# y-scope/pinot

Hardware: AMD Instinct MI355X
Metric: scanned rows/sec + achieved HBM GB/s, filtered SUM on 1B-row segment (higher is better)
Workload: dtype int64

## Files before the change

### pinot_amd/csrc/pg_engine.hip

```cpp
#include <hip/hip_runtime.h>

#include <algorithm>
#include <chrono>
#include <array>
#include <atomic>
#include <condition_variable>
#include <functional>
#include <memory>
#include <cmath>
#include <cstdarg>
#include <cstdio>
#include <cstdlib>
#include <cstring>
#include <limits>
#include <mutex>
#include <string>
#include <thread>
#include <vector>

#include "../../include/pinot_gpu.h"
#include "pg_device.h"
#include "pg_filter_stats.h"
#include "pg_filter_fsm.h"
#include "pg_fsm_kernels.h"
#include "pg_kernels.h"
#include "pg_launch.h"
#include "pg_rank_image.h"
#include "pg_raw_set_table.h"
#include "pg_hll.h"
#include "pg_set_pass_layout.h"
#include "pg_group_plan.h"
#include "pg_chunk_decode.h"

namespace {

using namespace pg;

thread_local std::string g_error;

pg_status fail(pg_status st, const char* fmt, ...) {
  char buf[1024];
  va_list ap;
  va_start(ap, fmt);
  vsnprintf(buf, sizeof(buf), fmt, ap);
  va_end(ap);
  g_error = buf;
  return st;
}

#define HIP_TRY(expr)                                                                                  \
  do {                                                                                                 \
    hipError_t _e = (expr);                                                                            \
    if (_e != hipSuccess)                                                                              \
      return fail(_e == hipErrorOutOfMemory ? PG_ERR_OUT_OF_MEMORY : PG_ERR_DEVICE, "%s failed: %s (%s:%d)", #expr, \
                  hipGetErrorString(_e), __FILE__, __LINE__);                                          \
  } while (0)

struct Engine {
  bool initialized = false;
  std::atomic<uint64_t> epoch{0};
  int device = 0;
  int blocks_per_cu = 0;
  bool raw64_coalesced = true;
  int wide_plane = -1;
  bool partition_stats_cache = true;
  bool partition_packed = true;
  bool plane_async = true;
  bool staged_h2d = true;
  long long exact_stats_docs = 64ll << 20;
  int flags = 0;
  bool use_dma = true;
  int value_plane = -1;
  int tile_steps = 0;
  bool double_buffer = false;
  bool direct_result = true;
  int fold_finalize = -1;
  int fold_one_counter = 1;
  bool poll_result = true;
  bool distinct_lds = true;
  bool collect = false;
  bool chunk_decode_host = false;
  bool percentile_lds = true;
  bool set_lds = true;
  bool lane_skip = true;
  bool batch_blocks_per_cu_forced = false;
  int batch_blocks_per_cu = 4;
  bool scan_raw = true;
  bool scan_raw_set = true;
  int scan_simple_valid = 1;
  int scan_simple_pipe = 1;
  int scan_simple_dma = 1;
  int dma_nt = -1;
  int dma_blocks_per_cu = 0;
  bool scan_simple = true;
  bool scan_sparse = true;
  bool lean_batch = true;
  bool partition_two_level = true;
  bool fsm_perm = true;
  int index_and_waves = 0;
  bool batch_index = true;
  bool index_gather = true;
  bool fsm_fused = true;
  bool fsm_stats = true;
  bool fsm_episodes = true;
  bool plan_cache = true;
  bool group_publish = true;
  bool batch_more = true;
  bool group_one_launch = true;
  bool batch_group = true;
  bool batch_hist = true;
  bool batch_launch = true;
  bool leap2 = true;
  int sparse_lanes = 32;
  bool plane_gcd = true;
  bool scan_private = true;
  bool group_private = true;
  int group_log_replicas = 3;
  bool group_pack = true;
  bool scan_typed_private = true;
  bool scan_narrow_single = true;
  bool scan_narrow = true;
  bool group_partition = true;
  long long partition_min_docs = 1ll << 22;
  unsigned long long group_table_bytes = 64ull << 30;
// ... 1648 lines not shown
  if (dev < 0 || dev >= g_engine.logical_devices) return fail(PG_ERR_INVALID_ARGUMENT, "device %d out of range (have %d)", dev, g_engine.logical_devices);
  g_engine.device = dev;
  g_engine.blocks_per_cu = config ? config->blocks_per_cu : 0;
  g_engine.flags = config ? config->flags : 0;
  const char* nodma = getenv("PINOT_GPU_NO_DMA");
  g_engine.use_dma = !(nodma && nodma[0] == '1');
  const char* vp = getenv("PINOT_GPU_VALUE_PLANE");
  g_engine.value_plane = vp ? atoi(vp) : -1;
  const char* db = getenv("PINOT_GPU_DOUBLE_BUFFER");
  g_engine.double_buffer = db && db[0] == '1';
  const char* drv = getenv("PINOT_GPU_DIRECT_RESULT");
  g_engine.direct_result = !(drv && drv[0] == '0');
  const char* ffz = getenv("PINOT_GPU_FOLD_FINALIZE");
  g_engine.fold_finalize = ffz ? (ffz[0] == '0' ? 0 : 1) : -1;
  const char* foc = getenv("PINOT_GPU_FOLD_ONE_COUNTER");
  g_engine.fold_one_counter = foc ? (foc[0] == '0' ? 0 : 1) : 1;
  const char* prs = getenv("PINOT_GPU_POLL_RESULT");
  g_engine.poll_result = !(prs && prs[0] == '0');
  const char* lsk = getenv("PINOT_GPU_LANE_SKIP");
  g_engine.lane_skip = !(lsk && lsk[0] == '0');
  const char* bbc = getenv("PINOT_GPU_BATCH_BLOCKS_PER_CU");
  g_engine.batch_blocks_per_cu_forced = bbc != nullptr;
  g_engine.batch_blocks_per_cu = (bbc && atoi(bbc) > 0) ? atoi(bbc) : 4;
  const char* ssp = getenv("PINOT_GPU_SCAN_SPARSE");
  g_engine.scan_sparse = !(ssp && ssp[0] == '0');
  const char* ssm = getenv("PINOT_GPU_SCAN_SIMPLE");
  g_engine.scan_simple = !(ssm && ssm[0] == '0');
  const char* ssv = getenv("PINOT_GPU_SCAN_SIMPLE_VALID");
  g_engine.scan_simple_valid = ssv ? (ssv[0] == '0' ? 0 : (ssv[0] == '2' ? 2 : 1)) : 1;
  const char* spp = getenv("PINOT_GPU_SCAN_SIMPLE_PIPE");
  g_engine.scan_simple_pipe = spp ? (spp[0] == '0' ? 0 : (spp[0] == '2' ? 2 : 1)) : 1;
  const char* sdm = getenv("PINOT_GPU_SCAN_SIMPLE_DMA");
  g_engine.scan_simple_dma = sdm ? (sdm[0] == '0' ? 0 : (sdm[0] == '2' ? 2 : 1)) : 1;
  const char* sdn = getenv("PINOT_GPU_SCAN_SIMPLE_DMA_NT");
  g_engine.dma_nt = sdn ? (sdn[0] == '0' ? 0 : 1) : -1;
  const char* sdb = getenv("PINOT_GPU_SCAN_SIMPLE_DMA_BLOCKS_PER_CU");
  g_engine.dma_blocks_per_cu = sdb && atoi(sdb) > 0 ? atoi(sdb) : 0;
  const char* srw = getenv("PINOT_GPU_SCAN_RAW");
  g_engine.scan_raw = !(srw && srw[0] == '0');
  const char* srs = getenv("PINOT_GPU_SCAN_RAW_SET");
  g_engine.scan_raw_set = !(srs && srs[0] == '0');
  const char* bla = getenv("PINOT_GPU_BATCH_LAUNCH");
  g_engine.batch_launch = !(bla && bla[0] == '0');
  auto env_on = [](const char* name) { const char* v = getenv(name); return !(v && v[0] == '0'); };
  g_engine.lean_batch = env_on("PINOT_GPU_LEAN_BATCH");
  g_engine.set_lds = env_on("PINOT_GPU_SET_LDS");
  g_engine.distinct_lds = env_on("PINOT_GPU_DISTINCT_LDS");
  g_engine.percentile_lds = env_on("PINOT_GPU_PERCENTILE_LDS");
  { const char* cv = getenv("PINOT_GPU_COLLECT"); g_engine.collect = cv != nullptr && cv[0] == '1'; }
  { const char* cd = getenv("PINOT_GPU_CHUNK_DECODE"); g_engine.chunk_decode_host = cd != nullptr && strcmp(cd, "host") == 0; }
  g_engine.partition_two_level = env_on("PINOT_GPU_PARTITION_TWO_LEVEL");
  g_engine.fsm_perm = env_on("PINOT_GPU_FSM_PERM");
  g_engine.fsm_stats = env_on("PINOT_GPU_FSM_STATS");
  g_engine.fsm_fused = env_on("PINOT_GPU_FSM_FUSED");
  g_engine.fsm_episodes = env_on("PINOT_GPU_FSM_EPISODES");
  g_engine.index_gather = env_on("PINOT_GPU_INDEX_GATHER");
  g_engine.batch_index = env_on("PINOT_GPU_BATCH_INDEX");
  { const char* iaw = getenv("PINOT_GPU_INDEX_AND_WAVES"); g_engine.index_and_waves = iaw ? std::max(-64, std::min(32, atoi(iaw))) : 0; }
  g_engine.group_one_launch = env_on("PINOT_GPU_GROUP_ONE_LAUNCH");
  g_engine.plan_cache = env_on("PINOT_GPU_PLAN_CACHE");
  g_engine.group_publish = env_on("PINOT_GPU_GROUP_PUBLISH");
  const char* bmo = getenv("PINOT_GPU_BATCH_MORE");
  g_engine.batch_more = !(bmo && bmo[0] == '0');
  const char* bgr = getenv("PINOT_GPU_BATCH_GROUP");
  g_engine.batch_group = !(bgr && bgr[0] == '0');
  const char* bhi = getenv("PINOT_GPU_BATCH_HIST");
// ... 874 lines not shown
}

static pg_status prepare_fsm_side(pg_segment* seg, ExecCtx* ctx, const pg::fstats::Fsm& fsm, FsmSide* side);
static pg_status device_fsm_filter_stats(pg_segment* seg, ExecCtx* ctx, const pg_query* q, const FsmSide& side, pg_result* out);
struct ExecTrace {
  std::chrono::steady_clock::time_point t[6];
  bool seen[6];
};
static thread_local ExecTrace t_exec_trace;
static bool exec_trace_on() { static const bool on = getenv("PINOT_GPU_EXEC_TRACE") != nullptr; return on; }
static inline void exec_mark(int i) {
  if (!exec_trace_on()) return;
  t_exec_trace.t[i] = std::chrono::steady_clock::now();
  t_exec_trace.seen[i] = true;
}

static pg_status execute_impl(pg_segment* seg, const pg_query* q, pg_result* out, unsigned long long* d_out_bitmap_request,
                              uint64_t* host_bitmap, int64_t host_bitmap_words, int64_t* out_cardinality, bool allow_metadata_plan = true,
                              Deferred* defer = nullptr, FsmSide* side = nullptr);

enum class ScanKernel { Hist, Narrow, NarrowSingle, Sparse, Simple, SimpleSet, SimpleValid, Raw, RawSet, PrivateFsm, Private, PrivateTyped, Distinct, GroupDistinct, Counts, GroupCounts, Collect, GroupCollect, Hll, GroupHll, Agg };
static const struct { int id; bool writes_leaves; } kScanKernels[] = {
  {PG_KERNEL_SCAN_HIST, true}, {PG_KERNEL_SCAN_NARROW, true}, {PG_KERNEL_SCAN_NARROW, false}, {PG_KERNEL_SCAN_SPARSE, false}, {PG_KERNEL_SCAN_SIMPLE, false},
  {PG_KERNEL_SCAN_SIMPLE, false}, {PG_KERNEL_SCAN_SIMPLE_VALID, false}, {PG_KERNEL_SCAN_RAW, false}, {PG_KERNEL_SCAN_RAW_SET, false}, {PG_KERNEL_SCAN_PRIVATE, false}, {PG_KERNEL_SCAN_PRIVATE, true},
  {PG_KERNEL_SCAN_PRIVATE_TYPED, true}, {PG_KERNEL_SCAN_DISTINCT, true}, {PG_KERNEL_GROUP_DISTINCT, true}, {PG_KERNEL_SCAN_COUNTS, true}, {PG_KERNEL_GROUP_COUNTS, true},
  {PG_KERNEL_SCAN_COLLECT, true}, {PG_KERNEL_GROUP_COLLECT, true}, {PG_KERNEL_SCAN_HLL, true}, {PG_KERNEL_GROUP_HLL, true}, {PG_KERNEL_SCAN_AGG, false}};
static_assert(sizeof(kScanKernels) / sizeof(kScanKernels[0]) == (size_t)ScanKernel::Agg + 1, "one row per ScanKernel");
struct ScanChoice {
  ScanKernel kernel = ScanKernel::Agg, general = ScanKernel::Agg;
  int hist_slot = -1, hist_cw = 0;
  bool hist_guarded = false;
  bool pipe = false;
  bool dma = false, dma_nt = false;
  int dma_blocks_per_cu = 0;
};
constexpr int kPipeMinSelectivityPct = 5;
constexpr int kDmaMinTilesPerWave = 8;
constexpr int kDmaMinSlotBytes = 6912;
constexpr int kDmaBlocksPerCu = 2;
constexpr long long kInfinityCacheBytes = 256ll << 20;
static void plan_scan_simple_dma(const pg_segment* seg, int filter_bits, int value_bits, bool dense, ScanChoice* k) {
  const int bpc = std::min(blocks_scan_simple_dma(filter_bits, value_bits, kLdsBudget), g_engine.dma_blocks_per_cu > 0 ? g_engine.dma_blocks_per_cu : kDmaBlocksPerCu);
  if (bpc < 1) return;
  k->dma_blocks_per_cu = bpc;
  const long long tiles = doc_tiles(seg), slot_bytes = 256ll * (filter_bits + value_bits);
  k->dma_nt = g_engine.dma_nt >= 0 ? g_engine.dma_nt == 1 : tiles * slot_bytes > kInfinityCacheBytes;
  const long long resident_waves = (long long)seg->num_cus * bpc * (kBlockThreads / 64);
  k->dma = g_engine.scan_simple_dma == 2 || (dense && slot_bytes >= kDmaMinSlotBytes && bpc >= kDmaBlocksPerCu && tiles >= kDmaMinTilesPerWave * resident_waves);
}
static ScanChoice choose_scan_kernel(const pg_segment* seg, const Lowered& lw, int hist_col, bool typed, bool want_bitmap, bool want_result) {
  const PlanParams& pl = lw.plan; const ScanParams& sp = lw.sp;
  const bool profile = (g_engine.flags & PG_CFG_PROFILE_WAVES) != 0;
  ScanChoice k;
  auto pick = [&k](ScanKernel kernel) { k.kernel = kernel; return k; };
  if (sp.num_nodes == 1 && sp.nodes[0].op == PG_FILTER_LEAF && sp.nodes[0].kind == kLeafRawSet) { k.general = ScanKernel::Private; return pick(ScanKernel::RawSet); }
  if (!lw.distinct_slots.empty() && lw.hll_pass) { k.general = ScanKernel::Private; return pick(lw.distinct_key_slots.empty() ? ScanKernel::Hll : ScanKernel::GroupHll); }
  if (!lw.distinct_slots.empty() && lw.collect_pass) { k.general = ScanKernel::Private; return pick(lw.distinct_key_slots.empty() ? ScanKernel::Collect : ScanKernel::GroupCollect); }
  if (!lw.distinct_slots.empty() && !lw.counts_pass) { k.general = ScanKernel::Private; return pick(lw.distinct_key_slots.empty() ? ScanKernel::Distinct : ScanKernel::GroupDistinct); }
  if (!lw.distinct_slots.empty()) { k.general = ScanKernel::Private; return pick(lw.distinct_key_slots.empty() ? ScanKernel::Counts : ScanKernel::GroupCounts); }
  bool private_leaves = true;
  for (int l = 0; l < pl.num_leaves; ++l) private_leaves &= pl.leaves[l].kind <= kLeafBitmap || pl.leaves[l].kind == kLeafDocRange;
  bool lane_private = g_engine.scan_private && !typed && !profile && private_leaves;
  for (int i = 0; i < pl.num_agg_cols && hist_col >= 0; ++i) if (lw.col_of_slot[(size_t)pl.agg_cols[i].col] == hist_col * 2) k.hist_slot = i;
  for (int i = 0; i < pl.num_agg_cols && lane_private; ++i) {
    const DevColumn& c = pl.cols[pl.agg_cols[i].col];
    lane_private = !c.is_raw && c.vkind == kValI32 && c.bits <= 31 && (!pl.agg_cols[i].need_sum || c.is_plane || i == k.hist_slot);
  }
  const bool hist = lane_private && k.hist_slot == 0 && pl.num_agg_cols == 1;
  if (k.hist_slot >= 0 && !hist) lane_private = false;
  bool lane_typed = g_engine.scan_private && g_engine.scan_typed_private && !lane_private && pl.num_agg_cols > 0 && !profile && private_leaves;
  for (int i = 0; i < pl.num_agg_cols && lane_typed; ++i) {
    const DevColumn& c = pl.cols[pl.agg_cols[i].col];
    lane_typed = c.is_raw || (c.vkind != kValI32 && c.bits <= 31);
  }
  k.general = k.kernel = lane_private ? ScanKernel::Private : (lane_typed ? ScanKernel::PrivateTyped : ScanKernel::Agg);
  if (hist) {
    k.hist_cw = hist_counter_bits(seg->cols[(size_t)hist_col]);
    k.hist_guarded = std::max(__atomic_load_n(&seg->cols[(size_t)hist_col].hist_tier, __ATOMIC_RELAXED), g_engine.hist_guard ? 1 : 0) >= 1 && k.hist_cw < 32;
// ... 171 lines not shown
      int bpc = std::max(1, std::min(waves_scan_raw_set(sp.nodes[0].lo_hi) / wpb, (int)(kLdsBudget / (g.lds + 1024))));
      if (tiles <= 2ll * seg->num_cus * bpc * wpb) bpc = std::min(bpc, 2);
      g.blocks = grid_blocks(seg, tiles, wpb, bpc);
      break;
    }
    case ScanKernel::Private: g.blocks = grid_blocks(seg, tiles, wpb, std::max(1, waves_scan_private(num_agg_cols) / wpb)); break;
    case ScanKernel::PrivateTyped: g.blocks = grid_blocks(seg, tiles, wpb, std::max(1, waves_scan_private_typed(num_agg_cols) / wpb)); break;
    default: g.blocks = geo.blocks; g.threads = geo.threads; g.lds = geo.lds; break;
  }
  return g;
}
static bool scan_batch_kind(const ScanChoice& k, int num_agg_cols, BatchKind* kind) {
  const bool lean = g_engine.lean_batch;
  switch (k.kernel) {
    case ScanKernel::Hist: *kind = k.hist_cw == 8 ? BatchKind::Hist8 : (k.hist_cw == 16 ? BatchKind::Hist16 : BatchKind::Hist32); return !k.hist_guarded && g_engine.batch_hist;
    case ScanKernel::Narrow: case ScanKernel::NarrowSingle: *kind = k.kernel == ScanKernel::Narrow ? BatchKind::Narrow : BatchKind::NarrowSingle; return g_engine.batch_more;
    case ScanKernel::Simple: case ScanKernel::SimpleSet: *kind = !lean ? BatchKind::Private : (k.kernel == ScanKernel::Simple ? BatchKind::Simple : BatchKind::SimpleSet); return true;
    case ScanKernel::Raw: *kind = !lean && k.general == ScanKernel::Private ? BatchKind::Private : BatchKind::Raw; return true;
    case ScanKernel::RawSet: return false;
    case ScanKernel::SimpleValid: return false;
    case ScanKernel::PrivateFsm: case ScanKernel::Private: *kind = BatchKind::Private; return true;
    case ScanKernel::PrivateTyped: *kind = num_agg_cols <= 1 ? BatchKind::Typed1 : (num_agg_cols == 2 ? BatchKind::Typed2 : BatchKind::TypedMax); return g_engine.batch_more;
    default: return false;
  }
}
static void launch_scan_kernel(const ScanChoice& k, const ScanGrid& g, int num_agg_cols, bool typed, hipStream_t stream, const ScanParams& sp) {
  const bool one = num_agg_cols <= 1;
  const int lean_threads = g.wide ? kWideBlockThreads : kBlockThreads;
  switch (k.kernel) {
    case ScanKernel::Hist: launch_scan_hist(k.hist_cw, k.hist_guarded, g.blocks, g.lds, stream, sp); break;
    case ScanKernel::Narrow: case ScanKernel::NarrowSingle: launch_scan_narrow(k.kernel == ScanKernel::NarrowSingle, g.blocks, stream, sp); break;
    case ScanKernel::Sparse: launch_scan_sparse(one, g.blocks, stream, sp); break;
    case ScanKernel::Simple: case ScanKernel::SimpleSet:
      if (k.dma) launch_scan_simple_dma(g.blocks, k.dma_nt, stream, sp);
      else if (k.pipe) launch_scan_simple_pipe(g.blocks, lean_threads, stream, sp);
      else launch_scan_simple(g.blocks, lean_threads, stream, sp, k.kernel == ScanKernel::SimpleSet);
      break;
    case ScanKernel::SimpleValid: launch_scan_simple_valid(g.blocks, lean_threads, stream, sp, g_engine.scan_simple_valid == 2); break;
    case ScanKernel::Raw: launch_scan_raw(g.blocks, lean_threads, stream, sp); break;
    case ScanKernel::RawSet: launch_scan_raw_set(sp.nodes[0].lo_hi, g.blocks, g.lds, stream, sp); break;
    case ScanKernel::PrivateFsm: launch_scan_private_fsm(num_agg_cols, g.blocks, stream, sp); break;
    case ScanKernel::Private: launch_scan_private(num_agg_cols, g.blocks, stream, sp); break;
    case ScanKernel::PrivateTyped: launch_scan_private_typed(num_agg_cols, g.blocks, stream, sp); break;
    case ScanKernel::Agg: launch_scan_agg(g_engine.use_dma, one, typed, g.blocks, g.threads, g.lds, stream, sp); break;
    case ScanKernel::Distinct: case ScanKernel::GroupDistinct: case ScanKernel::Counts: case ScanKernel::GroupCounts:
    case ScanKernel::Collect: case ScanKernel::GroupCollect: case ScanKernel::Hll: case ScanKernel::GroupHll: break;
  }
}
struct QueryRun {
  pg_segment* seg; const pg_query* q; pg_result* out; ExecCtx* ctx; Deferred* defer;
  int na, ng, hist_col = -1;
  bool want_bitmap, timed, stats_is_final = false;
  Lowered lw;
  PlaneHold planes;
  std::vector<int> projected;
  QueryRun(pg_segment* s, const pg_query* q_, pg_result* o, ExecCtx* c, Deferred* d, int na_, int ng_, bool want_bitmap_, bool timed_)
      : seg(s), q(q_), out(o), ctx(c), defer(d), na(na_), ng(ng_), want_bitmap(want_bitmap_), timed(timed_), planes(s, {}) {}
  void add_projected(int c) { if (std::find(projected.begin(), projected.end(), c) == projected.end()) projected.push_back(c); }
};
static pg_status defer_item(QueryRun& r, std::shared_ptr<LoweredItem> item) {
  item->plane_columns = r.planes.columns;
  item->doc_sets = r.lw.doc_sets;
  r.defer->item = std::move(item);
  r.defer->cacheable = !r.lw.plane_pending;
  r.defer->planes.reset(new PlaneHold(std::move(r.planes)));
  return kDeferred;
}
// ... 3427 lines not shown
```

### pinot_amd/csrc/pg_launch.h

```cpp
#ifndef PG_LAUNCH_H
#define PG_LAUNCH_H
#include <hip/hip_runtime.h>

#include <algorithm>

#include "pg_device.h"

namespace pg {

template <typename K>
int max_waves_per_cu(K kernel) {
  hipFuncAttributes attr;
  if (hipFuncGetAttributes(&attr, reinterpret_cast<const void*>(kernel)) != hipSuccess || attr.numRegs <= 0) return 16;
  const int alloc = ((attr.numRegs + 7) / 8) * 8;
  return std::max(1, std::min(6, 512 / alloc)) * 4;
}
template <typename K>
int max_waves_per_cu_lean(K kernel) {
  hipFuncAttributes attr;
  if (hipFuncGetAttributes(&attr, reinterpret_cast<const void*>(kernel)) != hipSuccess || attr.numRegs <= 0) return 16;
  const int alloc = ((attr.numRegs + 7) / 8) * 8;
  return std::max(1, std::min(8, 512 / alloc)) * 4;
}
template <typename K>
void set_dynamic_lds(K kernel, size_t bytes) {
  if (bytes > 48 * 1024) (void)hipFuncSetAttribute(reinterpret_cast<const void*>(kernel), hipFuncAttributeMaxDynamicSharedMemorySize, (int)bytes);
}

void launch_scan_agg(bool dma, bool one_slot, bool typed, int blocks, int threads, size_t lds, hipStream_t stream, const ScanParams& p);
int waves_scan_agg(bool one_slot, bool typed);
void launch_scan_private(int agg_cols, int blocks, hipStream_t stream, const ScanParams& p);
int waves_scan_private(int agg_cols);
void launch_scan_private_fsm(int agg_cols, int blocks, hipStream_t stream, const ScanParams& p);
int waves_scan_private_fsm(int agg_cols);
void launch_scan_private_batch(bool one_slot, int total_blocks, hipStream_t stream, const ScanParams* items, const uint32_t* block_first, int num_items);
void launch_scan_sparse(bool one_slot, int blocks, hipStream_t stream, const ScanParams& p);
int waves_scan_sparse(bool one_slot);
void launch_scan_simple(int blocks, int threads, hipStream_t stream, const ScanParams& p, bool set_leaf = false);
int waves_scan_simple();
bool scan_simple_pipe_shape(int filter_bits, int value_bits);
void launch_scan_simple_pipe(int blocks, int threads, hipStream_t stream, const ScanParams& p);
int waves_scan_simple_pipe();
constexpr int kDmaSlots = 2;
size_t scan_simple_dma_lds(int filter_bits, int value_bits);
void launch_scan_simple_dma(int blocks, bool nt, hipStream_t stream, const ScanParams& p);
int blocks_scan_simple_dma(int filter_bits, int value_bits, size_t lds_budget);
void launch_scan_simple_valid(int blocks, int threads, hipStream_t stream, const ScanParams& p, bool skip_empty_tiles);
int waves_scan_simple_valid();
void launch_scan_raw(int blocks, int threads, hipStream_t stream, const ScanParams& p);
int waves_scan_raw();
void launch_scan_raw_set(int key_bytes, int blocks, size_t table_bytes, hipStream_t stream, const ScanParams& p);
int waves_scan_raw_set(int key_bytes);
void launch_raw_set_bitmap(int key_bytes, int blocks, hipStream_t stream, const RawSetBitmapParams& p);
int waves_raw_set_bitmap(int key_bytes);
void launch_scan_lean_batch(int kind, int total_blocks, hipStream_t stream, const ScanParams* items, const uint32_t* block_first, int num_items);
int waves_scan_lean_batch(int kind);
void launch_scan_narrow(bool single_leaf, int blocks, hipStream_t stream, const ScanParams& p);
int waves_scan_narrow(bool single_leaf);
void launch_scan_narrow_batch(bool single_leaf, int total_blocks, hipStream_t stream, const ScanParams* items, const uint32_t* block_first, int num_items);
int waves_scan_narrow_batch(bool single_leaf);
void launch_scan_typed_batch(int agg_slots, int total_blocks, hipStream_t stream, const ScanParams* items, const uint32_t* block_first, int num_items);
int waves_scan_typed_batch(int agg_slots);
void launch_index_and_kernel(int blocks, hipStream_t stream, const IndexAndParams& ap, uint32_t num_windows);
int waves_index_and();
int index_and_batch_blocks_per_cu();
int index_and_batch_block_waves();
void launch_index_and_batch(int total_blocks, hipStream_t stream, const IndexAndParams* items, const uint32_t* block_first, int num_items);
void launch_scan_group(bool dma, bool lds_table, int blocks, int threads, size_t lds, hipStream_t stream, const GroupParams& gp);
int waves_scan_group();
void launch_group_private(bool lds_table, int blocks, int threads, size_t lds, hipStream_t stream, const GroupParams& gp);
int waves_group_private();
void launch_group_lds_batch(int total_blocks, int threads, size_t lds, hipStream_t stream, const GroupParams* items, const uint32_t* block_first, int num_items);
int waves_group_lds_batch();

void launch_scan_hist(int counter_bits, bool guarded, int blocks, size_t lds, hipStream_t stream, const ScanParams& p);
int waves_scan_hist(int counter_bits, bool guarded);
void launch_scan_hist_batch(int counter_bits, int total_blocks, size_t lds, hipStream_t stream, const ScanParams* items, const uint32_t* block_first, int num_items);
int waves_scan_hist_batch(int counter_bits);
// ... 56 lines not shown
```

### pinot_amd/csrc/pg_scan_simple_dma.h

```cpp
#pragma once
#include "pg_scan_simple.h"

namespace pg {

typedef const __attribute__((address_space(3))) uint32_t* LdsWords;

constexpr int kDmaRecordBytes = 1024;
static_assert(sizeof(BlockPartial) * (kBlockThreads / 64) + 16 <= kDmaRecordBytes, "the records and the flag fit their area");
__host__ __device__ constexpr int dma_slot_bytes(int filter_bits, int value_bits) { return 256 * (filter_bits + value_bits); }
__host__ __device__ constexpr size_t dma_lds_bytes(int filter_bits, int value_bits, int slots, int waves) {
  return (size_t)kDmaRecordBytes + (size_t)waves * slots * dma_slot_bytes(filter_bits, value_bits);
}

template <int J> __device__ __forceinline__ void dma_wait() { asm volatile("s_waitcnt vmcnt(%0)" :: "n"(J) : "memory"); }

template <int N, int kAux>
__device__ __forceinline__ void dma_stage_tile(const uint8_t* f_tile, const uint8_t* v_tile, int f_bytes, int v_bytes, int nf, uint8_t* slot, int lane) {
#pragma unroll
  for (int j = 0; j < N; ++j) {
    const bool is_f = j < nf;
    const int at = (is_f ? j : j - nf) * 1024, chunk = is_f ? f_bytes : v_bytes;
    const uint8_t* src = (is_f ? f_tile : v_tile) + at + lane * 16;
    uint8_t* dst = slot + (is_f ? 0 : f_bytes) + at;
    if (at + lane * 16 < chunk)
      __builtin_amdgcn_global_load_lds((const __attribute__((address_space(1))) void*)src, (__attribute__((address_space(3))) void*)dst, 16, 0, kAux);
  }
}

template <typename P>
__device__ __forceinline__ void dma_tile(const P& p, long long tile, int lane, const uint8_t* slot, unsigned long long& count, unsigned long long& sum,
                                         uint32_t& umin, uint32_t& umax) {
  const auto& L = p.nodes[0];
  const auto& ac = p.agg_cols[0];
  const LdsWords fw = (LdsWords)(const uint32_t*)slot + lane * L.bits;
  const LdsWords vw = (LdsWords)(const uint32_t*)(slot + 256 * L.bits) + lane * ac.bits;
  uint32_t m = L.lo == 0 ? simple_range_dispatch<true>(L.bits, fw, 0u, L.span) : simple_range_dispatch<false>(L.bits, fw, (uint32_t)L.lo, L.span);
  if (L.exclusive) m = ~m;
  const long long rem = (long long)p.num_docs - (tile * 2048 + lane * 32);
  m &= rem >= 32 ? 0xFFFFFFFFu : (rem <= 0 ? 0u : ((1u << (int)rem) - 1u));
  count += (unsigned)__builtin_popcount(m);
  uint32_t psum = 0, tmin = 0xFFFFFFFFu, tmax = 0u;
  unsigned long long wsum = 0;
  simple_agg_dispatch(ac.bits, vw, m, ac.need_sum != 0, ac.need_minmax != 0, psum, wsum, tmin, tmax);
  sum += wsum + psum;
  umin = tmin < umin ? tmin : umin;
// ... 20 lines not shown
  const long long first = (long long)block_index * waves_per_block + wave_in_block;
  const long long n = first < num_tiles ? (num_tiles - first + total_waves - 1) / total_waves : 0;
#pragma unroll
  for (int k = 0; k < S - 1; ++k)
    if (k < n) dma_stage_tile<N, kAux>(L.fwd + (first + k * total_waves) * f_bytes, ac.fwd + (first + k * total_waves) * v_bytes, f_bytes, v_bytes, nf, ring + k * slot_bytes, lane);
  long long i = 0, tile = first;
  int rd = 0, wr = S - 1;
  for (; i + (S - 1) < n; ++i, tile += total_waves) {
    asm volatile("s_waitcnt lgkmcnt(0)" ::: "memory");
    const long long ahead = tile + (S - 1) * total_waves;
    dma_stage_tile<N, kAux>(L.fwd + ahead * f_bytes, ac.fwd + ahead * v_bytes, f_bytes, v_bytes, nf, ring + wr * slot_bytes, lane);
    dma_wait<N * (S - 1)>();
    dma_tile(p, tile, lane, ring + rd * slot_bytes, count, sum, umin, umax);
    rd = rd + 1 == S ? 0 : rd + 1;
    wr = wr + 1 == S ? 0 : wr + 1;
  }
#define PG_DMA_DRAIN(R) if (S - 1 >= R && n - i == R) { dma_wait<N * (R - 1)>(); dma_tile(p, tile, lane, ring + rd * slot_bytes, count, sum, umin, umax); \
                          rd = rd + 1 == S ? 0 : rd + 1; ++i; tile += total_waves; }
  PG_DMA_DRAIN(3) PG_DMA_DRAIN(2) PG_DMA_DRAIN(1)
#undef PG_DMA_DRAIN
  static_assert(S <= 4, "PG_DMA_DRAIN covers rings of up to four slots");

  BlockPartial mine;
  partial_identity(mine);
  mine.count = (unsigned long long)wave_sum_i64((long long)count);
  mine.sum[0] = wave_sum_i64((long long)sum);
  mine.kmin[0] = wave_min_i32(umin == 0xFFFFFFFFu ? 0x7FFFFFFF : (int32_t)umin);
  mine.kmax[0] = wave_max_i32(count == 0ull ? (int32_t)0x80000000 : (int32_t)umax);
  if (lane == 0) red[wave_in_block] = mine;
  __syncthreads();
  publish_block_partial(p, red, waves_per_block, fold_flag_ptr, block_index, num_blocks);
}


}
```

### pinot_amd/csrc/pg_unit_scan_simple_dma.hip

```cpp
#include "pg_scan_simple_dma.h"
#include "pg_launch.h"

namespace pg {

template <int N, int kAux>
__global__ __launch_bounds__(kBlockThreads) void scan_simple_dma_kernel(const ScanParams p) {
  extern __shared__ __attribute__((aligned(16))) uint8_t dma_lds[];
  scan_simple_dma_body<N, kDmaSlots, kAux>(p, blockIdx.x, gridDim.x, dma_lds);
}

typedef void (*DmaKernel)(const ScanParams);
static_assert((kSimpleMaxBits + 3) / 4 == 5, "N = 2 .. 10");
#define K(N) {scan_simple_dma_kernel<N, 0>, scan_simple_dma_kernel<N, 2>}
static const DmaKernel kDmaKernels[9][2] = {K(2), K(3), K(4), K(5), K(6), K(7), K(8), K(9), K(10)};
#undef K

size_t scan_simple_dma_lds(int filter_bits, int value_bits) { return dma_lds_bytes(filter_bits, value_bits, kDmaSlots, kBlockThreads / 64); }

void launch_scan_simple_dma(int blocks, bool nt, hipStream_t stream, const ScanParams& p) {
  const int n = (p.nodes[0].bits + 3) / 4 + (p.agg_cols[0].bits + 3) / 4;
  const DmaKernel kernel = kDmaKernels[n - 2][nt ? 1 : 0];
  static bool raised[9][2];
  bool& done = raised[n - 2][nt ? 1 : 0];
  if (!done) { set_dynamic_lds(kernel, scan_simple_dma_lds(kSimpleMaxBits, kSimpleMaxBits)); done = true; }
  kernel<<<dim3((unsigned)blocks), dim3((unsigned)kBlockThreads), scan_simple_dma_lds(p.nodes[0].bits, p.agg_cols[0].bits), stream>>>(p);
}

int blocks_scan_simple_dma(int filter_bits, int value_bits, size_t lds_budget) {
  static const int reg_waves = [] {
    int least = max_waves_per_cu_lean(kDmaKernels[0][0]);
    for (int n = 0; n < 9; ++n) for (int a = 0; a < 2; ++a) least = std::min(least, max_waves_per_cu_lean(kDmaKernels[n][a]));
    return least;
  }();
  return std::min(reg_waves / (kBlockThreads / 64), (int)(lds_budget / scan_simple_dma_lds(filter_bits, value_bits)));
}

}
```

Measured before the change: 1850 billion.

## Specialize DMA scan kernel per filter/value bit-width pair

Measured after the change: 1932 billion (median of 6 runs). +4.4%, better.

```diff
diff --git a/pinot_amd/csrc/host/check/dma_pairs_main.cpp b/pinot_amd/csrc/host/check/dma_pairs_main.cpp
--- /dev/null
+++ b/pinot_amd/csrc/host/check/dma_pairs_main.cpp
@@ -0,0 +1,85 @@
+#include <cstdint>
+#include <cstdio>
+#include <vector>
+
+#include "../../pg_dma_pairs.h"
+
+static int failures = 0;
+#define EXPECT(cond) do { if (!(cond)) { fprintf(stderr, "%s:%d: %s\n", __FILE__, __LINE__, #cond); ++failures; } } while (0)
+
+using namespace pg;
+
+struct Piece { int column, at, lanes; };
+static std::vector<Piece> stage_tile_at_run_time(int filter_bits, int value_bits, std::vector<int>& slot_writes) {
+  const int f_bytes = 256 * filter_bits, v_bytes = 256 * value_bits, nf = (filter_bits + 3) >> 2;
+  const int n = (filter_bits + 3) / 4 + (value_bits + 3) / 4;
+  std::vector<Piece> out;
+  slot_writes.assign((size_t)f_bytes + v_bytes, 0);
+  for (int j = 0; j < n; ++j) {
+    const bool is_f = j < nf;
+    const int at = (is_f ? j : j - nf) * 1024, chunk = is_f ? f_bytes : v_bytes;
+    int lanes = 0;
+    for (int lane = 0; lane < 64; ++lane) {
+      if (at + lane * 16 < chunk) {
+        ++lanes;
+        const int dst = (is_f ? 0 : f_bytes) + at + lane * 16;
+        for (int b = 0; b < 16; ++b) ++slot_writes.at((size_t)dst + b);
+      }
+    }
+    out.push_back(Piece{is_f ? 0 : 1, at, lanes});
+  }
+  return out;
+}
+
+int main() {
+  std::vector<int> seen((size_t)kDmaPairs, 0);
+  int admitted = 0;
+  for (int f = 0; f <= kDmaMaxBits + 1; ++f)
+    for (int v = 0; v <= kDmaMaxBits + 1; ++v) {
+      const bool in_rule = f >= 1 && f <= kDmaMaxBits && v >= 1 && v <= kDmaMaxBits && f + v >= 27 && f + v <= 38;
+      EXPECT(dma_pair_admitted(f, v) == in_rule);
+      const int at = dma_pair_index(f, v);
+      if (!in_rule) { EXPECT(at == -1); continue; }
+      ++admitted;
+      EXPECT(at >= 0 && at < kDmaPairs);
+      if (at >= 0 && at < kDmaPairs) {
+        ++seen[(size_t)at];
+        EXPECT(dma_pair_at(at) == f * 32 + v);
+      }
+      EXPECT(dma_slot_bytes(f, v) >= kDmaMinSlotBytes);
+      EXPECT(2 * dma_lds_bytes(f, v, kDmaSlotsPerWave, kDmaWavesPerBlock) <= kDmaLdsBudget);
+    }
+  EXPECT(admitted == kDmaPairs && kDmaPairs == 102);
+  for (int at = 0; at < kDmaPairs; ++at) EXPECT(seen[(size_t)at] == 1);
+  EXPECT(dma_pair_at(-1) == 0 && dma_pair_at(kDmaPairs) == 0);
+  EXPECT(dma_pair_index(10, 17) >= 0 && dma_pair_index(6, 20) == -1 && dma_pair_index(19, 20) == -1 && dma_pair_index(20, 19) == -1 && dma_pair_index(20, 6) == -1);
+  EXPECT(dma_slot_bytes(10, 17) == 6912 && dma_lds_bytes(10, 17, 2, 4) == 56320 && dma_lds_bytes(18, 20, 2, 4) == 78848);
+
+  for (int f = 1; f <= kDmaMaxBits; ++f)
+    for (int v = 1; v <= kDmaMaxBits; ++v) {
+      std::vector<int> writes;
+      const std::vector<Piece> run = stage_tile_at_run_time(f, v, writes);
+      EXPECT((int)run.size() == dma_instructions(f, v));
+      EXPECT(dma_instructions(f, v) >= 2 && dma_instructions(f, v) <= 10);
+      for (const int w : writes) EXPECT(w == 1);
+      size_t j = 0;
+      for (int column = 0; column < 2; ++column) {
+        const int bits = column == 0 ? f : v;
+        EXPECT(dma_pieces(bits) >= 1 && dma_pieces(bits) <= 5);
+        for (int piece = 0; piece < dma_pieces(bits) && j < run.size(); ++piece, ++j) {
+          const int base = piece >= 4 ? 4096 : 0, off = (piece & 3) * 1024;
+          EXPECT(off <= 4095);
+          EXPECT(run[j].column == column && run[j].at == base + off);
+          EXPECT(run[j].lanes == (piece + 1 < dma_pieces(bits) ? 64 : dma_last_lanes(bits)));
+        }
+        const int last = dma_last_lanes(bits);
+        EXPECT(last == 16 || last == 32 || last == 48 || last == 64);
+        EXPECT((dma_pieces(bits) - 1) * 1024 + last * 16 == 256 * bits);
+      }
+      EXPECT(j == run.size());
+    }
+
+  if (failures != 0) { fprintf(stderr, "dma_pairs: %d expectation(s) failed\n", failures); return 1; }
+  printf("ok\n");
+  return 0;
+}
diff --git a/pinot_amd/csrc/pg_dma_pairs.h b/pinot_amd/csrc/pg_dma_pairs.h
--- /dev/null
+++ b/pinot_amd/csrc/pg_dma_pairs.h
@@ -0,0 +1,54 @@
+#pragma once
+#include <cstddef>
+
+namespace pg {
+
+constexpr int kDmaMaxBits = 20;
+constexpr int kDmaSlotsPerWave = 2;
+constexpr int kDmaWavesPerBlock = 4;
+constexpr int kDmaRecordBytes = 1024;
+constexpr size_t kDmaLdsBudget = 156 * 1024;
+constexpr int kDmaMinSlotBytes = 6912;
+constexpr int kDmaBlocksPerCu = 2;
+
+constexpr int dma_pieces(int bits) { return (bits + 3) / 4; }
+constexpr int dma_last_lanes(int bits) { return 16 * (bits - 4 * (dma_pieces(bits) - 1)); }
+constexpr int dma_instructions(int filter_bits, int value_bits) { return dma_pieces(filter_bits) + dma_pieces(value_bits); }
+constexpr int dma_slot_bytes(int filter_bits, int value_bits) { return 256 * (filter_bits + value_bits); }
+constexpr size_t dma_lds_bytes(int filter_bits, int value_bits, int slots, int waves) {
+  return (size_t)kDmaRecordBytes + (size_t)waves * slots * dma_slot_bytes(filter_bits, value_bits);
+}
+
+constexpr bool dma_width(int bits) { return bits >= 1 && bits <= kDmaMaxBits; }
+constexpr bool dma_pair_admitted(int filter_bits, int value_bits) {
+  return dma_width(filter_bits) && dma_width(value_bits) && dma_slot_bytes(filter_bits, value_bits) >= kDmaMinSlotBytes &&
+         kDmaLdsBudget / dma_lds_bytes(filter_bits, value_bits, kDmaSlotsPerWave, kDmaWavesPerBlock) >= (size_t)kDmaBlocksPerCu;
+}
+constexpr int dma_pair_index(int filter_bits, int value_bits) {
+  if (!dma_pair_admitted(filter_bits, value_bits)) return -1;
+  int at = 0;
+  for (int f = 1; f <= kDmaMaxBits; ++f)
+    for (int v = 1; v <= kDmaMaxBits; ++v) {
+      if (f == filter_bits && v == value_bits) return at;
+      if (dma_pair_admitted(f, v)) ++at;
+    }
+  return -1;
+}
+constexpr int dma_pair_count() {
+  int n = 0;
+  for (int f = 1; f <= kDmaMaxBits; ++f)
+    for (int v = 1; v <= kDmaMaxBits; ++v) n += dma_pair_admitted(f, v) ? 1 : 0;
+  return n;
+}
+constexpr int kDmaPairs = dma_pair_count();
+constexpr int dma_pair_at(int index) {
+  int at = 0;
+  for (int f = 1; f <= kDmaMaxBits; ++f)
+    for (int v = 1; v <= kDmaMaxBits; ++v)
+      if (dma_pair_admitted(f, v) && at++ == index) return f * 32 + v;
+  return 0;
+}
+static_assert(kDmaPairs == 102, "27 <= f + v <= 38, both up to 20 bits");
+static_assert(dma_pair_admitted(10, 17) && dma_pair_admitted(7, 20) && dma_pair_admitted(20, 18) && !dma_pair_admitted(6, 20) && !dma_pair_admitted(19, 20), "the rule's edges");
+
+}
diff --git a/pinot_amd/csrc/pg_engine.hip b/pinot_amd/csrc/pg_engine.hip
--- a/pinot_amd/csrc/pg_engine.hip
+++ b/pinot_amd/csrc/pg_engine.hip
@@ -30,6 +30,7 @@
 #include "pg_hll.h"
 #include "pg_set_pass_layout.h"
 #include "pg_group_plan.h"
+#include "pg_dma_pairs.h"
 #include "pg_chunk_decode.h"
 
 namespace {
@@ -90,6 +91,7 @@
   int scan_simple_valid = 1;
   int scan_simple_pipe = 1;
   int scan_simple_dma = 1;
+  int dma_pair = 1;
   int dma_nt = -1;
   int dma_blocks_per_cu = 0;
   bool scan_simple = true;
@@ -1804,6 +1806,8 @@
   g_engine.scan_simple_pipe = spp ? (spp[0] == '0' ? 0 : (spp[0] == '2' ? 2 : 1)) : 1;
   const char* sdm = getenv("PINOT_GPU_SCAN_SIMPLE_DMA");
   g_engine.scan_simple_dma = sdm ? (sdm[0] == '0' ? 0 : (sdm[0] == '2' ? 2 : 1)) : 1;
+  const char* sdp = getenv("PINOT_GPU_SCAN_SIMPLE_DMA_PAIR");
+  g_engine.dma_pair = sdp && sdp[0] == '0' ? 0 : 1;
   const char* sdn = getenv("PINOT_GPU_SCAN_SIMPLE_DMA_NT");
   g_engine.dma_nt = sdn ? (sdn[0] == '0' ? 0 : 1) : -1;
   const char* sdb = getenv("PINOT_GPU_SCAN_SIMPLE_DMA_BLOCKS_PER_CU");
@@ -2744,18 +2748,19 @@
   bool hist_guarded = false;
   bool pipe = false;
   bool dma = false, dma_nt = false;
+  bool dma_pair = false;
   int dma_blocks_per_cu = 0;
 };
 constexpr int kPipeMinSelectivityPct = 5;
 constexpr int kDmaMinTilesPerWave = 8;
-constexpr int kDmaMinSlotBytes = 6912;
-constexpr int kDmaBlocksPerCu = 2;
+static_assert(kDmaLdsBudget == kLdsBudget, "pg_dma_pairs.h prices the rings against this budget");
 constexpr long long kInfinityCacheBytes = 256ll << 20;
 static void plan_scan_simple_dma(const pg_segment* seg, int filter_bits, int value_bits, bool dense, ScanChoice* k) {
   const int bpc = std::min(blocks_scan_simple_dma(filter_bits, value_bits, kLdsBudget), g_engine.dma_blocks_per_cu > 0 ? g_engine.dma_blocks_per_cu : kDmaBlocksPerCu);
   if (bpc < 1) return;
   k->dma_blocks_per_cu = bpc;
-  const long long tiles = doc_tiles(seg), slot_bytes = 256ll * (filter_bits + value_bits);
+  const long long tiles = doc_tiles(seg), slot_bytes = dma_slot_bytes(filter_bits, value_bits);
+  k->dma_pair = g_engine.dma_pair != 0 && scan_simple_dma_pair_shape(filter_bits, value_bits);
   k->dma_nt = g_engine.dma_nt >= 0 ? g_engine.dma_nt == 1 : tiles * slot_bytes > kInfinityCacheBytes;
   const long long resident_waves = (long long)seg->num_cus * bpc * (kBlockThreads / 64);
   k->dma = g_engine.scan_simple_dma == 2 || (dense && slot_bytes >= kDmaMinSlotBytes && bpc >= kDmaBlocksPerCu && tiles >= kDmaMinTilesPerWave * resident_waves);
@@ -2993,7 +2998,7 @@
     case ScanKernel::Narrow: case ScanKernel::NarrowSingle: launch_scan_narrow(k.kernel == ScanKernel::NarrowSingle, g.blocks, stream, sp); break;
     case ScanKernel::Sparse: launch_scan_sparse(one, g.blocks, stream, sp); break;
     case ScanKernel::Simple: case ScanKernel::SimpleSet:
-      if (k.dma) launch_scan_simple_dma(g.blocks, k.dma_nt, stream, sp);
+      if (k.dma) launch_scan_simple_dma(g.blocks, k.dma_nt, k.dma_pair, stream, sp);
       else if (k.pipe) launch_scan_simple_pipe(g.blocks, lean_threads, stream, sp);
       else launch_scan_simple(g.blocks, lean_threads, stream, sp, k.kernel == ScanKernel::SimpleSet);
       break;
diff --git a/pinot_amd/csrc/pg_launch.h b/pinot_amd/csrc/pg_launch.h
--- a/pinot_amd/csrc/pg_launch.h
+++ b/pinot_amd/csrc/pg_launch.h
@@ -43,7 +43,13 @@
 int waves_scan_simple_pipe();
 constexpr int kDmaSlots = 2;
 size_t scan_simple_dma_lds(int filter_bits, int value_bits);
-void launch_scan_simple_dma(int blocks, bool nt, hipStream_t stream, const ScanParams& p);
+bool scan_simple_dma_pair_shape(int filter_bits, int value_bits);
+typedef void (*DmaKernel)(const ScanParams);
+constexpr int kDmaPairParts = 3;
+DmaKernel scan_simple_dma_pair_part0(int at, bool nt);
+DmaKernel scan_simple_dma_pair_part1(int at, bool nt);
+DmaKernel scan_simple_dma_pair_part2(int at, bool nt);
+void launch_scan_simple_dma(int blocks, bool nt, bool pair, hipStream_t stream, const ScanParams& p);
 int blocks_scan_simple_dma(int filter_bits, int value_bits, size_t lds_budget);
 void launch_scan_simple_valid(int blocks, int threads, hipStream_t stream, const ScanParams& p, bool skip_empty_tiles);
 int waves_scan_simple_valid();
diff --git a/pinot_amd/csrc/pg_scan_simple_dma.h b/pinot_amd/csrc/pg_scan_simple_dma.h
--- a/pinot_amd/csrc/pg_scan_simple_dma.h
+++ b/pinot_amd/csrc/pg_scan_simple_dma.h
@@ -1,16 +1,13 @@
 #pragma once
+#include "pg_dma_pairs.h"
 #include "pg_scan_simple.h"
 
 namespace pg {
 
 typedef const __attribute__((address_space(3))) uint32_t* LdsWords;
 
-constexpr int kDmaRecordBytes = 1024;
 static_assert(sizeof(BlockPartial) * (kBlockThreads / 64) + 16 <= kDmaRecordBytes, "the records and the flag fit their area");
-__host__ __device__ constexpr int dma_slot_bytes(int filter_bits, int value_bits) { return 256 * (filter_bits + value_bits); }
-__host__ __device__ constexpr size_t dma_lds_bytes(int filter_bits, int value_bits, int slots, int waves) {
-  return (size_t)kDmaRecordBytes + (size_t)waves * slots * dma_slot_bytes(filter_bits, value_bits);
-}
+static_assert(kDmaMaxBits == kSimpleMaxBits && kDmaWavesPerBlock == kBlockThreads / 64, "pg_dma_pairs.h speaks of this kernel's widths and workgroups");
 
 template <int J> __device__ __forceinline__ void dma_wait() { asm volatile("s_waitcnt vmcnt(%0)" :: "n"(J) : "memory"); }
 
@@ -97,5 +94,114 @@
   publish_block_partial(p, red, waves_per_block, fold_flag_ptr, block_index, num_blocks);
 }
 
-
-}
+template <int B, int J, int kAux>
+__device__ __forceinline__ void dma_stage_piece(const uint8_t* src, uint8_t* dst, int lane) {
+  constexpr int base = J >= 4 ? 4096 : 0, off = (J & 3) * 1024;
+  if (J + 1 < dma_pieces(B) || dma_last_lanes(B) == 64 || lane < dma_last_lanes(B))
+    __builtin_amdgcn_global_load_lds((const __attribute__((address_space(1))) void*)(src + base), (__attribute__((address_space(3))) void*)(dst + base), 16, off, kAux);
+}
+template <int B, int kAux>
+__device__ __forceinline__ void dma_stage_column(const uint8_t* src, uint8_t* dst, int lane) {
+  static_assert(dma_pieces(B) <= 5, "columns of up to 20 bits");
+  dma_stage_piece<B, 0, kAux>(src, dst, lane);
+  if constexpr (dma_pieces(B) > 1) dma_stage_piece<B, 1, kAux>(src, dst, lane);
+  if constexpr (dma_pieces(B) > 2) dma_stage_piece<B, 2, kAux>(src, dst, lane);
+  if constexpr (dma_pieces(B) > 3) dma_stage_piece<B, 3, kAux>(src, dst, lane);
+  if constexpr (dma_pieces(B) > 4) dma_stage_piece<B, 4, kAux>(src, dst, lane);
+}
+
+template <int FB, int VB, bool kLoZero, bool kMinMax>
+__device__ __forceinline__ void dma_pair_tile(const uint8_t* slot, int lane, uint32_t lo, uint32_t span, uint32_t flip, long long rem,
+                                              unsigned long long& count, unsigned long long& sum, uint32_t& umin, uint32_t& umax) {
+  const LdsWords fw = (LdsWords)(const uint32_t*)slot + lane * FB;
+  const LdsWords vw = (LdsWords)(const uint32_t*)(slot + 256 * FB) + lane * VB;
+  uint32_t fd[FB], vd[VB];
+#pragma unroll
+  for (int i = 0; i < FB; ++i) fd[i] = fw[i];
+#pragma unroll
+  for (int i = 0; i < VB; ++i) vd[i] = vw[i];
+  uint32_t m = 0;
+  range16_private<FB, 0, kLoZero>((const uint32_t*)fd, lo, span, m);
+  range16_private<FB, 1, kLoZero>((const uint32_t*)fd, lo, span, m);
+  m = __builtin_bitreverse32(m) ^ flip;
+  m &= rem >= 32 ? 0xFFFFFFFFu : (rem <= 0 ? 0u : ((1u << (int)rem) - 1u));
+  count += (unsigned)__builtin_popcount(m);
+  uint32_t psum = 0, tmin = 0xFFFFFFFFu, tmax = 0u;
+  unsigned long long wsum = 0;
+  agg16_private<VB, 0>((const uint32_t*)vd, m, true, kMinMax, psum, wsum, tmin, tmax);
+  agg16_private<VB, 1>((const uint32_t*)vd, m, true, kMinMax, psum, wsum, tmin, tmax);
+  sum += wsum + psum;
+  umin = tmin < umin ? tmin : umin;
+  umax = tmax > umax ? tmax : umax;
+}
+
+template <int FB, int VB, int kAux, bool kLoZero, bool kMinMax, typename P>
+__device__ __forceinline__ void dma_pair_tiles(const P& p, long long first, uint32_t n, long long total_waves, uint8_t* ring, int lane,
+                                               unsigned long long& count, unsigned long long& sum, uint32_t& umin, uint32_t& umax) {
+  constexpr int f_bytes = 256 * FB, v_bytes = 256 * VB, slot_bytes = f_bytes + v_bytes, N = dma_instructions(FB, VB);
+  const auto& L = p.nodes[0];
+  const uint32_t lo = (uint32_t)L.lo, span = L.span, flip = L.exclusive ? 0xFFFFFFFFu : 0u;
+  const uint32_t lane_at = (uint32_t)lane * 16u;
+  const uint8_t* f_next = L.fwd + first * f_bytes;
+  const uint8_t* v_next = p.agg_cols[0].fwd + first * v_bytes;
+  const long long f_step = total_waves * f_bytes, v_step = total_waves * v_bytes;
+  long long rem = (long long)p.num_docs - (first * 2048 + lane * 32);
+  const long long rem_step = total_waves * 2048;
+  if (n > 0) {
+    dma_stage_column<FB, kAux>(f_next + lane_at, ring, lane);
+    dma_stage_column<VB, kAux>(v_next + lane_at, ring + f_bytes, lane);
+  }
+  int rd = 0;
+  for (uint32_t i = 0; i < n; ++i, rem -= rem_step) {
+    if (i + 1 < n) {
+      asm volatile("s_waitcnt lgkmcnt(0)" ::: "memory");
+      f_next += f_step; v_next += v_step;
+      uint8_t* wr = ring + (slot_bytes - rd);
+      dma_stage_column<FB, kAux>(f_next + lane_at, wr, lane);
+      dma_stage_column<VB, kAux>(v_next + lane_at, wr + f_bytes, lane);
+      dma_wait<N>();
+    } else {
+      dma_wait<0>();
+    }
+    dma_pair_tile<FB, VB, kLoZero, kMinMax>(ring + rd, lane, lo, span, flip, rem, count, sum, umin, umax);
+    rd = slot_bytes - rd;
+  }
+}
+
+template <int FB, int VB, int kAux, typename P>
+__device__ __forceinline__ void scan_simple_dma_pair_body(const P& p, uint32_t block_index, uint32_t num_blocks, uint8_t* lds) {
+  static_assert(kDmaSlotsPerWave == 2 && dma_instructions(FB, VB) <= 63, "two slots; vmcnt counts to 63");
+  BlockPartial* red = reinterpret_cast<BlockPartial*>(lds);
+  uint32_t* fold_flag_ptr = reinterpret_cast<uint32_t*>(lds + sizeof(BlockPartial) * (kBlockThreads / 64));
+  const int lane = threadIdx.x & 63;
+  const int wave_in_block = __builtin_amdgcn_readfirstlane((int)(threadIdx.x >> 6));
+  const int waves_per_block = blockDim.x >> 6;
+  const long long total_waves = (long long)num_blocks * waves_per_block;
+  const long long num_tiles = ((long long)p.num_docs + 2047) / 2048;
+  uint8_t* ring = lds + kDmaRecordBytes + (size_t)wave_in_block * kDmaSlotsPerWave * dma_slot_bytes(FB, VB);
+
+  unsigned long long count = 0, sum = 0;
+  uint32_t umin = 0xFFFFFFFFu, umax = 0u;
+  const long long first = (long long)block_index * waves_per_block + wave_in_block;
+  const uint32_t n = first < num_tiles ? (uint32_t)((num_tiles - first + total_waves - 1) / total_waves) : 0u;
+  const bool lo_zero = p.nodes[0].lo == 0, need_sum = p.agg_cols[0].need_sum != 0, need_minmax = p.agg_cols[0].need_minmax != 0;
+#define PG_PAIR_TILES(Z, M) dma_pair_tiles<FB, VB, kAux, Z, M>(p, first, n, total_waves, ring, lane, count, sum, umin, umax)
+  if (lo_zero) { if (need_sum && !need_minmax) PG_PAIR_TILES(true, false); else PG_PAIR_TILES(true, true); }
+  else { if (need_sum && !need_minmax) PG_PAIR_TILES(false, false); else PG_PAIR_TILES(false, true); }
+#undef PG_PAIR_TILES
+  if (!need_sum) sum = 0;
+  if (!need_minmax) { umin = 0xFFFFFFFFu; umax = 0u; }
+
+  BlockPartial mine;
+  partial_identity(mine);
+  mine.count = (unsigned long long)wave_sum_i64((long long)count);
+  mine.sum[0] = wave_sum_i64((long long)sum);
+  mine.kmin[0] = wave_min_i32(umin == 0xFFFFFFFFu ? 0x7FFFFFFF : (int32_t)umin);
+  mine.kmax[0] = wave_max_i32(count == 0ull ? (int32_t)0x80000000 : (int32_t)umax);
+  if (lane == 0) red[wave_in_block] = mine;
+  __syncthreads();
+  publish_block_partial(p, red, waves_per_block, fold_flag_ptr, block_index, num_blocks);
+}
+
+
+}
diff --git a/pinot_amd/csrc/pg_scan_simple_dma_pair_part.h b/pinot_amd/csrc/pg_scan_simple_dma_pair_part.h
--- /dev/null
+++ b/pinot_amd/csrc/pg_scan_simple_dma_pair_part.h
@@ -0,0 +1,31 @@
+#include <utility>
+
+#include "pg_scan_simple_dma.h"
+#include "pg_launch.h"
+
+namespace pg {
+
+template <int FB, int VB, int kAux>
+__global__ __launch_bounds__(kBlockThreads) void scan_simple_dma_pair_kernel(const ScanParams p) {
+  extern __shared__ __attribute__((aligned(16))) uint8_t dma_lds[];
+  scan_simple_dma_pair_body<FB, VB, kAux>(p, blockIdx.x, gridDim.x, dma_lds);
+}
+
+namespace {
+constexpr int kPart = PG_DMA_PAIR_PART;
+static_assert(kPart >= 0 && kPart < kDmaPairParts, "pg_launch.h declares the parts");
+constexpr int kPartPairs = (kDmaPairs - kPart + kDmaPairParts - 1) / kDmaPairParts;
+struct PartTable { DmaKernel at[kPartPairs][2]; };
+constexpr int part_pair(size_t i) { return dma_pair_at((int)i * kDmaPairParts + kPart); }
+template <size_t... I>
+constexpr PartTable part_table(std::index_sequence<I...>) {
+  return PartTable{{{scan_simple_dma_pair_kernel<part_pair(I) / 32, part_pair(I) % 32, 0>, scan_simple_dma_pair_kernel<part_pair(I) / 32, part_pair(I) % 32, 2>}...}};
+}
+const PartTable kPartTable = part_table(std::make_index_sequence<kPartPairs>());
+}
+
+#define PG_DMA_PAIR_PART_NAME2(P) scan_simple_dma_pair_part##P
+#define PG_DMA_PAIR_PART_NAME(P) PG_DMA_PAIR_PART_NAME2(P)
+DmaKernel PG_DMA_PAIR_PART_NAME(PG_DMA_PAIR_PART)(int at, bool nt) { return kPartTable.at[at / kDmaPairParts][nt ? 1 : 0]; }
+
+}
diff --git a/pinot_amd/csrc/pg_unit_scan_simple_dma.hip b/pinot_amd/csrc/pg_unit_scan_simple_dma.hip
--- a/pinot_amd/csrc/pg_unit_scan_simple_dma.hip
+++ b/pinot_amd/csrc/pg_unit_scan_simple_dma.hip
@@ -9,7 +9,6 @@
   scan_simple_dma_body<N, kDmaSlots, kAux>(p, blockIdx.x, gridDim.x, dma_lds);
 }
 
-typedef void (*DmaKernel)(const ScanParams);
 static_assert((kSimpleMaxBits + 3) / 4 == 5, "N = 2 .. 10");
 #define K(N) {scan_simple_dma_kernel<N, 0>, scan_simple_dma_kernel<N, 2>}
 static const DmaKernel kDmaKernels[9][2] = {K(2), K(3), K(4), K(5), K(6), K(7), K(8), K(9), K(10)};
@@ -17,7 +16,30 @@
 
 size_t scan_simple_dma_lds(int filter_bits, int value_bits) { return dma_lds_bytes(filter_bits, value_bits, kDmaSlots, kBlockThreads / 64); }
 
-void launch_scan_simple_dma(int blocks, bool nt, hipStream_t stream, const ScanParams& p) {
+static_assert(kDmaSlots == kDmaSlotsPerWave, "pg_dma_pairs.h prices the rings this unit launches");
+
+bool scan_simple_dma_pair_shape(int filter_bits, int value_bits) { return dma_pair_index(filter_bits, value_bits) >= 0; }
+
+static DmaKernel dma_pair_kernel(int at, bool nt) {
+  static_assert(kDmaPairParts == 3, "one case per unit");
+  switch (at % kDmaPairParts) {
+    case 0: return scan_simple_dma_pair_part0(at, nt);
+    case 1: return scan_simple_dma_pair_part1(at, nt);
+    default: return scan_simple_dma_pair_part2(at, nt);
+  }
+}
+
+void launch_scan_simple_dma(int blocks, bool nt, bool pair, hipStream_t stream, const ScanParams& p) {
+  if (pair) {
+    const int at = dma_pair_index(p.nodes[0].bits, p.agg_cols[0].bits);
+    const DmaKernel kernel = dma_pair_kernel(at, nt);
+    static bool raised[kDmaPairs][2];
+    bool& done = raised[at][nt ? 1 : 0];
+    const size_t lds = scan_simple_dma_lds(p.nodes[0].bits, p.agg_cols[0].bits);
+    if (!done) { set_dynamic_lds(kernel, lds); done = true; }
+    kernel<<<dim3((unsigned)blocks), dim3((unsigned)kBlockThreads), lds, stream>>>(p);
+    return;
+  }
   const int n = (p.nodes[0].bits + 3) / 4 + (p.agg_cols[0].bits + 3) / 4;
   const DmaKernel kernel = kDmaKernels[n - 2][nt ? 1 : 0];
   static bool raised[9][2];
diff --git a/pinot_amd/csrc/pg_unit_scan_simple_dma_pair0.hip b/pinot_amd/csrc/pg_unit_scan_simple_dma_pair0.hip
--- /dev/null
+++ b/pinot_amd/csrc/pg_unit_scan_simple_dma_pair0.hip
@@ -0,0 +1,2 @@
+#define PG_DMA_PAIR_PART 0
+#include "pg_scan_simple_dma_pair_part.h"
diff --git a/pinot_amd/csrc/pg_unit_scan_simple_dma_pair1.hip b/pinot_amd/csrc/pg_unit_scan_simple_dma_pair1.hip
--- /dev/null
+++ b/pinot_amd/csrc/pg_unit_scan_simple_dma_pair1.hip
@@ -0,0 +1,2 @@
+#define PG_DMA_PAIR_PART 1
+#include "pg_scan_simple_dma_pair_part.h"
diff --git a/pinot_amd/csrc/pg_unit_scan_simple_dma_pair2.hip b/pinot_amd/csrc/pg_unit_scan_simple_dma_pair2.hip
--- /dev/null
+++ b/pinot_amd/csrc/pg_unit_scan_simple_dma_pair2.hip
@@ -0,0 +1,2 @@
+#define PG_DMA_PAIR_PART 2
+#include "pg_scan_simple_dma_pair_part.h"
```
